# Schatten2021/rust-raytracing

Measured on AMD Instinct MI355X. Metric: Mrays/s (primary rays, whole node), 10k-sphere 1080p 64spp, higher is better.
Workload: dtype f64; 1 GPU; C2: 10k random spheres (scene seed 1), 1920x1080, 64 spp; width=1920, height=1080, rays_per_pixel=64, n_objects=10000, partition=single GPU

## Files before the change

rust-raytracing_amd/csrc/rtx_api.hip:

```cpp
#include "../../include/rtx_hip.h"
#include "rtx_launch.h"

#include <cmath>
#include <cstdio>
#include <cstdlib>
#include <cstring>
#include <string>
#include <thread>
#include <vector>

using namespace rtx;

namespace {

thread_local std::string g_last_error;

int32_t fail(RtxStatus st, const std::string &msg)
{
    g_last_error = msg;
    return (int32_t)st;
}

#define RTX_HIP_CHECK(expr)                                                                              \
    do {                                                                                                 \
        hipError_t e_ = (expr);                                                                          \
        if (e_ != hipSuccess)                                                                            \
            return fail(e_ == hipErrorOutOfMemory ? RTX_ERR_OUT_OF_MEMORY : RTX_ERR_HIP,                 \
                        std::string(#expr) + ": " + hipGetErrorString(e_));                              \
    } while (0)

bool device_is_gfx950(int dev)
{
    hipDeviceProp_t prop;
    if (hipGetDeviceProperties(&prop, dev) != hipSuccess) return false;
    return std::strncmp(prop.gcnArchName, "gfx950", 6) == 0;
}

int usable_device_count()
{
    int n = 0;
    if (hipGetDeviceCount(&n) != hipSuccess) { (void)hipGetLastError(); return 0; }
    int ok = 0;
    for (int d = 0; d < n; ++d) ok += device_is_gfx950(d) ? 1 : 0;
    return ok;
}

constexpr size_t kDefaultScratchBytes = (size_t)24576 << 20;

uint32_t tri_leaf_size(bool plain, uint32_t tuning)
{
    const uint32_t t = (tuning >> RTX_TUNE_TRI_LEAF_SHIFT) & 15u;
    const uint32_t v = t ? t : (plain ? 5u : 2u);
    return v > kQNodeLeafMax ? kQNodeLeafMax : v;
}

bool debug_prints()
{
    static const bool on = std::getenv("RTX_HIP_DEBUG") != nullptr;
    return on;
}

}

#ifndef RTX_GRABS_PER_WAVE
#define RTX_GRABS_PER_WAVE 16
#endif

constexpr uint64_t kHalvesBelowRays = 0;

struct RtxSceneHandle_ {
    int device = 0;
    int n_cus = 0;
    RtxConfig cfg{};
    RtxCamera cam{};
    SceneView sv{};
    std::vector<RtxObject> objects;
    std::vector<void *> scene_allocs;
    double *samples = nullptr;  size_t samples_bytes = 0;
    double *acc = nullptr;      size_t acc_bytes = 0;
    double *tables = nullptr;   size_t tables_doubles = 0;
    double *h_tables = nullptr; size_t h_tables_doubles = 0;
    double *state = nullptr;    size_t state_bytes = 0;
    void *wf_state = nullptr;   size_t wf_bytes = 0;
    void *pool = nullptr;       size_t pool_bytes = 0;
    void *slots = nullptr;      size_t slots_bytes = 0;
    void *tile_lists = nullptr; size_t tile_lists_bytes = 0;
    PathStep *transcript = nullptr; uint32_t *transcript_counts = nullptr; uint32_t transcript_steps = 0;
    Counters *counters = nullptr;
    unsigned long long *work_counter = nullptr;
    SceneView *d_sv = nullptr;  bool sv_dirty = true;
    RowsView *d_rv = nullptr;
    hipEvent_t ev[4] = { nullptr, nullptr, nullptr, nullptr };
    struct SecondHalf {
        hipStream_t stream = nullptr;
        hipEvent_t fork = nullptr, join = nullptr, stage1_done = nullptr;
        Counters *counters = nullptr, *counters_stage1 = nullptr;
        unsigned long long *work_counter = nullptr;
        RowsView *d_rv = nullptr;
        double *state = nullptr;    size_t state_bytes = 0;
        void *queue = nullptr;      size_t queue_bytes = 0;
    } half2;
    Counters *counters_stage1 = nullptr;
    size_t scratch_limit = 0;
    hipStream_t last_stream = nullptr;
    bool have_last_stream = false;
    hipEvent_t ev_done = nullptr;
    bool have_done = false;
    unsigned long long *h_watchdog = nullptr;
    hipEvent_t ev_watchdog = nullptr;
    bool watchdog_pending = false;
    uint32_t t_w = 0, t_h = 0, t_rb = 0, t_rs = 0, t_blk = 0, t_nr = 0;
    double t_fov = 0.0;
    bool t_valid = false;
};

namespace {

template <class T>
int32_t upload_vec(RtxSceneHandle_ *h, const std::vector<T> &v, const T **out)
{
    *out = nullptr;
    if (v.empty()) return RTX_OK;
    void *d = nullptr;
    RTX_HIP_CHECK(hipMalloc(&d, v.size() * sizeof(T)));
    h->scene_allocs.push_back(d);
    RTX_HIP_CHECK(hipMemcpy(d, v.data(), v.size() * sizeof(T), hipMemcpyHostToDevice));
    *out = static_cast<const T *>(d);
    return RTX_OK;
}

// ... 573 lines not shown
    hipStream_t stream = static_cast<hipStream_t>(stream_);
    if (stats) std::memset(stats, 0, sizeof *stats);
    if (n_rows == 0 || width == 0) return RTX_OK;
    if (!d_out_rgb) return fail(RTX_ERR_INVALID_ARGUMENT, "rtx_render_rows: null output");
    if ((uint64_t)n_rows * width > 0xFFFFFFF0ull) return fail(RTX_ERR_INVALID_ARGUMENT, "rtx_render_rows: more than 2^32 pixels per call");
    RTX_HIP_CHECK(hipSetDevice(h->device));
    if (int32_t rc = check_watchdog(h, false)) return rc;
    if (int32_t rc = adopt_stream(h, stream)) return rc;
    struct DoneGuard {
        RtxSceneHandle_ *h; hipStream_t stream;
        ~DoneGuard() {
            if (hipEventRecord(h->ev_done, stream) == hipSuccess) h->have_done = true;
            else { (void)hipGetLastError(); (void)hipDeviceSynchronize(); h->have_done = false; }
        }
    } done_guard{h, stream};

    const uint32_t npix = n_rows * width;
    const uint64_t spp = h->cfg.rays_per_pixel;
    if (h->sv.n_objects == 0 && spp > 0) {
        RTX_HIP_CHECK(hipMemsetAsync(d_out_rgb, 0, (size_t)npix * 3 * sizeof(double), stream));
        if (stats) {
            RTX_HIP_CHECK(hipStreamSynchronize(stream));
            stats->primary_rays = (uint64_t)npix * spp;
            stats->kernel = h->cfg.kernel;
        }
        return RTX_OK;
    }
    const uint64_t outside_tree = ((h->sv.bvh_flags & 1u) ? 0u : h->sv.n_spheres) +
                                  (uint64_t)(h->sv.n_tri_filter - h->sv.n_tri_tree);
    uint32_t kernel = h->cfg.kernel;
    const uint32_t tuning = h->cfg.tuning;
    const bool want_tiles = (tuning & RTX_TUNE_NO_TILES) == 0u, classic = (tuning & RTX_TUNE_BVH_CLASSIC) != 0u;
    if (kernel == RTX_KERNEL_AUTO) {
        if (h->sv.n_bvh_nodes != 0 && outside_tree <= 64) {
            const bool mesh = (h->sv.bvh_flags & 2u) != 0u && h->sv.n_tri_tree >= 1024u;
            kernel = mesh ? RTX_KERNEL_BVH_REGROUP : RTX_KERNEL_BVH;
            if (mesh && (uint64_t)npix * spp >= (1ull << 20) && want_tiles && wavefront_mesh_supported(h->sv, true))
                kernel = RTX_KERNEL_WAVEFRONT;
        } else {
            kernel = RTX_KERNEL_MIXED;
        }
    }

#ifndef RTX_LAB
    if (kernel == RTX_KERNEL_BVH || kernel == RTX_KERNEL_BVH_REGROUP || kernel == RTX_KERNEL_WAVEFRONT) {
        const bool sphere_tree = h->sv.n_bvh_nodes != 0 && (h->sv.bvh_flags & 19u) == 17u;
        const bool tri_tree = h->sv.n_bvh_nodes != 0 && (h->sv.bvh_flags & 2u) != 0u;
        if (sphere_tree) kernel = RTX_KERNEL_BVH;
        else if (!tri_tree) kernel = RTX_KERNEL_MIXED;
        else if (kernel == RTX_KERNEL_BVH) kernel = RTX_KERNEL_BVH_REGROUP;
    }
#endif
    const bool wf_mesh = wavefront_mesh_supported(h->sv, want_tiles);
    const bool wf_spheres = kLabBuild && !wf_mesh && h->sv.n_bvh_nodes != 0 && (h->sv.bvh_flags & 3u) == 1u;
    if (kernel == RTX_KERNEL_WAVEFRONT && !wf_mesh && !wf_spheres) kernel = RTX_KERNEL_BVH_REGROUP;
    const bool tiled = (kernel == RTX_KERNEL_BVH || kernel == RTX_KERNEL_BVH_REGROUP || kernel == RTX_KERNEL_WAVEFRONT) && want_tiles;
    const uint32_t tiles_x = tiled ? (width + 7u) / 8u : 0u;
    const uint64_t per_sample64 = tiled ? (uint64_t)tiles_x * ((n_rows + 7u) / 8u) * 64u : (uint64_t)npix;
    if (per_sample64 > 0xFFFFFFF0ull) return fail(RTX_ERR_INVALID_ARGUMENT, "rtx_render_rows: more than 2^32 ray slots per sample");
    const uint32_t per_sample = (uint32_t)per_sample64;
    uint64_t batch = spp;
    uint64_t tile_list_bytes = 0;
    {
        const bool sph2 = kernel == RTX_KERNEL_BVH && (h->sv.bvh_flags & 2u) == 0u && h->sv.n_bvh_nodes != 0;
        const uint64_t per_ray = 4 * sizeof(double) + (kernel == RTX_KERNEL_WAVEFRONT ? wavefront_state_bytes(1u << 20, 1) >> 20 : 0) +
                                 (sph2 ? 64 + 5 : 0);
        size_t cap_bytes = h->scratch_limit ? h->scratch_limit : kDefaultScratchBytes;
        size_t free_b = 0, total_b = 0;
        if (hipMemGetInfo(&free_b, &total_b) == hipSuccess) {
            const size_t mine = h->samples_bytes + h->wf_bytes + h->tile_lists_bytes;
            const size_t avail = (free_b + mine) / 4 * 3;
            if (cap_bytes > avail) cap_bytes = avail;
        } else (void)hipGetLastError();
        if ((tuning & RTX_TUNE_NO_TILE_LISTS) == 0u && tiled) {
            if (sph2) tile_list_bytes = bvh_spheres_tile_list_bytes(per_sample64);
            else if (kernel == RTX_KERNEL_WAVEFRONT && wf_mesh) tile_list_bytes = wavefront_tile_list_bytes(per_sample64);
            if (tile_list_bytes > cap_bytes / 4) tile_list_bytes = 0;
        }
        const uint64_t fixed = tile_list_bytes +
                               (sph2 ? (uint64_t)bvh_spheres_queue_bytes(0, h->n_cus) + bvh_spheres_spill_bytes(h->sv, h->n_cus) : 0) +
                               (kernel == RTX_KERNEL_WAVEFRONT ? (uint64_t)wavefront_state_bytes(0, 1) + wavefront_spill_bytes(h->sv, h->n_cus) : 0) +
                               (kernel == RTX_KERNEL_MIXED || kernel == RTX_KERNEL_MIXED_VERIFY ? (uint64_t)mixed_state_bytes(h->n_cus) : 0);
        const uint64_t room = cap_bytes > fixed ? cap_bytes - fixed : 0;
        const uint64_t fit = room / (per_sample64 * per_ray);
        const uint64_t fit32 = 0xFFFFFFF0ull / per_sample64;
        if (batch > fit) batch = fit ? fit : 1;
        if (batch > fit32) batch = fit32;
    }

    if (int32_t rc = ensure_tables(h, width, height, row_begin, row_stride, row_block, n_rows, stream)) return rc;

    if (spp > 0) {
        if (int32_t rc = grow((void **)&h->samples, &h->samples_bytes, (size_t)(batch * per_sample64 * 4 * sizeof(double)))) return rc;
    }
    if (batch < spp) {
        if (int32_t rc = grow((void **)&h->acc, &h->acc_bytes, (size_t)npix * 3 * sizeof(double))) return rc;
    }
    const bool spheres_kernel = kernel == RTX_KERNEL_BVH && (h->sv.bvh_flags & 2u) == 0u && h->sv.n_bvh_nodes != 0 && !classic;
    const bool mesh_kernel = kernel == RTX_KERNEL_BVH_REGROUP && (h->sv.bvh_flags & 2u) != 0u && !classic;
#ifdef RTX_LAB
    const bool pool_kernel = kernel == RTX_KERNEL_BVH_REGROUP && (h->sv.bvh_flags & 3u) == 1u && h->sv.n_bvh_nodes != 0 && !classic;
#endif
    if (kernel == RTX_KERNEL_BVH || kernel == RTX_KERNEL_BVH_REGROUP) {
#ifdef RTX_LAB
        const size_t need = pool_kernel ? bvh_spheres_pool_bytes(h->sv, h->n_cus)
                            : spheres_kernel ? bvh_spheres_spill_bytes(h->sv, h->n_cus)
                            : mesh_kernel ? bvh_mesh_spill_bytes(h->sv, h->n_cus) : bvh_spill_bytes(h->sv, h->n_cus);
#else
        if (!spheres_kernel && !mesh_kernel) return fail(RTX_ERR_HIP, "internal: no tree kernel for this scene (product dispatch)");
        const size_t need = spheres_kernel ? bvh_spheres_spill_bytes(h->sv, h->n_cus) : bvh_mesh_spill_bytes(h->sv, h->n_cus);
#endif
        if (int32_t rc = grow((void **)&h->state, &h->state_bytes, need)) return rc;
    }
    if (kernel == RTX_KERNEL_MIXED || kernel == RTX_KERNEL_MIXED_VERIFY) {
        if (int32_t rc = grow((void **)&h->state, &h->state_bytes, mixed_state_bytes(h->n_cus))) return rc;
    }
    const bool spheres_two_stage = spheres_kernel && h->cfg.max_bounces > 0 && (tuning & RTX_TUNE_ONE_STAGE) == 0u &&
                                   (batch * per_sample64 >= (1ull << 20) || (tuning & RTX_TUNE_TWO_STAGE) != 0u) &&
                                   bvh_spheres_two_stage_ok(h->sv, tiled);
#ifdef RTX_LAB
    const bool stage2_slots = spheres_two_stage && (tuning & RTX_TUNE_STAGE2_SLOTS) != 0u && (h->sv.bvh_flags & 16u) != 0u &&
                              (tuning & (RTX_TUNE_NO_QNODES | RTX_TUNE_INLINE_LEAVES | RTX_TUNE_STAGE2_POOL | RTX_TUNE_STAGE2_PAIR)) == 0u;
    if (stage2_slots) {
        if (int32_t rc = grow(&h->slots, &h->slots_bytes, bvh_spheres_slots_bytes(h->n_cus))) return rc;
    }
#else
    const bool stage2_slots = false;
#endif
    if (spheres_two_stage) {
        if (int32_t rc = grow(&h->wf_state, &h->wf_bytes, bvh_spheres_queue_bytes(batch * per_sample64, h->n_cus))) return rc;
        if (tile_list_bytes != 0)
            if (int32_t rc = grow(&h->tile_lists, &h->tile_lists_bytes, (size_t)tile_list_bytes)) return rc;
#ifdef RTX_LAB
        if (tuning & (RTX_TUNE_STAGE2_POOL | RTX_TUNE_STAGE2_PAIR)) {
            const size_t a = bvh_spheres_pool2_bytes(h->n_cus), b = bvh_spheres_pair_bytes(h->n_cus);
            if (int32_t rc = grow(&h->pool, &h->pool_bytes, a > b ? a : b)) return rc;
        }
#endif
    }
    if (kernel == RTX_KERNEL_WAVEFRONT) {
#ifdef RTX_LAB
        const size_t need = wf_mesh ? wavefront_spill_bytes(h->sv, h->n_cus) : wavefront_spheres_spill_bytes(h->sv, h->n_cus);
#else
        const size_t need = wavefront_spill_bytes(h->sv, h->n_cus);
#endif
        if (int32_t rc = grow((void **)&h->state, &h->state_bytes, need)) return rc;
        if (int32_t rc = grow(&h->wf_state, &h->wf_bytes, wavefront_state_bytes(batch * per_sample64, wavefront_levels(h->sv)))) return rc;
        if (wf_mesh && tile_list_bytes != 0)
            if (int32_t rc = grow(&h->tile_lists, &h->tile_lists_bytes, (size_t)tile_list_bytes)) return rc;
    }

    RowsView rv{};
    rv.width = width; rv.height = height;
    rv.row_begin = row_begin; rv.row_stride = row_stride; rv.n_rows = n_rows; rv.row_block = row_block;
    rv.npix = npix;
    rv.div_width = make_fastdiv(width); rv.div_row_block = make_fastdiv(row_block); rv.div_npix = make_fastdiv(npix);
    rv.div_tiles_x = make_fastdiv(tiles_x); rv.div_per_sample = make_fastdiv(per_sample);
    rv.sin_x = h->tables; rv.cos_x = h->tables + width;
    rv.sin_y = h->tables + 2 * (size_t)width; rv.cos_y = rv.sin_y + n_rows;

    if (h->sv_dirty) {
        RTX_HIP_CHECK(hipMemcpyAsync(h->d_sv, &h->sv, sizeof(SceneView), hipMemcpyHostToDevice, stream));
        h->sv_dirty = false;
    }
    RTX_HIP_CHECK(hipMemsetAsync(h->counters, 0, sizeof(Counters) * kCounterShards, stream));
    float trace_ms = 0.f, resolve_ms = 0.f, stage1_ms = 0.f;
    unsigned long long s1_exact = 0, s1_filter = 0, s1_box = 0, prev_exact = 0, prev_filter = 0, prev_box = 0;
    uint32_t launches = 0;

    if (spp == 0) {
        rv.n_samples = 0; rv.n_rays = 0; rv.tiles_x = 0;
        RTX_HIP_CHECK(launch_resolve(nullptr, nullptr, d_out_rgb, rv, npix, 0, true, true, stream));
    }
    const uint32_t sph_flags = ((tuning & RTX_TUNE_NO_PACKETS) ? 1u : 0u) | ((tuning & RTX_TUNE_SORT_SURVIVORS) ? 2u : 0u) |
                               ((tuning & RTX_TUNE_STAGE2_POOL) ? 4u : 0u) | ((tuning & RTX_TUNE_STAGE2_PAIR) ? 8u : 0u);
#ifdef RTX_LAB
    const bool halves_can = spheres_two_stage && batch == spp && spp >= 2 && !stage2_slots &&
                            (tuning & (RTX_TUNE_STAGE2_POOL | RTX_TUNE_STAGE2_PAIR)) == 0u;
#else
    const bool halves_can = spheres_two_stage && batch == spp && spp >= 2;
#endif
    const bool halves = halves_can && (tuning & RTX_TUNE_NO_HALVES) == 0u &&
                        ((tuning & RTX_TUNE_HALVES) != 0u || per_sample64 * spp <= kHalvesBelowRays);
    if (halves) {
        auto &b = h->half2;
        if (!b.stream) {
            int least = 0, greatest = 0;
            RTX_HIP_CHECK(hipDeviceGetStreamPriorityRange(&least, &greatest));
            RTX_HIP_CHECK(hipStreamCreateWithPriority(&b.stream, hipStreamNonBlocking, least));
            RTX_HIP_CHECK(hipEventCreateWithFlags(&b.fork, hipEventDisableTiming));
            RTX_HIP_CHECK(hipEventCreateWithFlags(&b.join, hipEventDisableTiming));
            RTX_HIP_CHECK(hipEventCreate(&b.stage1_done));
            RTX_HIP_CHECK(hipMalloc((void **)&b.counters, sizeof(Counters) * kCounterShards));
            RTX_HIP_CHECK(hipMalloc((void **)&b.counters_stage1, sizeof(Counters) * kCounterShards));
            RTX_HIP_CHECK(hipMalloc((void **)&b.work_counter, sizeof(unsigned long long)));
            RTX_HIP_CHECK(hipMalloc((void **)&b.d_rv, sizeof(RowsView)));
        }
        const uint64_t ns[2] = { (spp + 1) / 2, spp / 2 };
        if (int32_t rc = grow((void **)&b.state, &b.state_bytes, bvh_spheres_spill_bytes(h->sv, h->n_cus))) return rc;
        if (int32_t rc = grow(&b.queue, &b.queue_bytes, bvh_spheres_queue_bytes(ns[1] * per_sample64, h->n_cus))) return rc;
        struct Join {
            RtxSceneHandle_ *h; hipStream_t main; bool forked = false;
            ~Join() {
                if (!forked) return;
                if (hipEventRecord(h->half2.join, h->half2.stream) != hipSuccess || hipStreamWaitEvent(main, h->half2.join, 0) != hipSuccess) {
                    (void)hipGetLastError(); (void)hipStreamSynchronize(h->half2.stream);
                }
            }
        } join{h, stream};
        RTX_HIP_CHECK(hipMemsetAsync(b.counters, 0, sizeof(Counters) * kCounterShards, stream));
        if (stats) RTX_HIP_CHECK(hipEventRecord(h->ev[0], stream));
        RTX_HIP_CHECK(hipEventRecord(b.fork, stream));
        RTX_HIP_CHECK(hipStreamWaitEvent(b.stream, b.fork, 0));
        join.forked = true;
        RowsView rvk[2] = { rv, rv };
        for (int k = 0; k < 2; ++k) {
            RowsView &r = rvk[k];
            r.sample_begin = k == 0 ? 0u : (uint32_t)ns[0];
            r.n_samples = (uint32_t)ns[k];
            r.n_rays = per_sample64 * ns[k];
            r.tiles_x = tiles_x;
            const uint64_t per_wave = r.n_rays / ((uint64_t)h->n_cus * 16u * (RTX_GRABS_PER_WAVE / 2));
            r.grab = (uint32_t)(per_wave >= 512 ? 512 : (per_wave <= 64 ? 64 : (per_wave & ~(uint64_t)63)));
            hipStream_t st = k == 0 ? stream : b.stream;
            RTX_HIP_CHECK(hipMemcpyAsync(k == 0 ? h->d_rv : b.d_rv, &r, sizeof(RowsView), hipMemcpyHostToDevice, st));
            RTX_HIP_CHECK(hipMemsetAsync(k == 0 ? h->work_counter : b.work_counter, 0, sizeof(unsigned long long), st));
            RTX_HIP_CHECK(launch_trace_bvh_spheres(h->d_sv, h->sv, k == 0 ? h->d_rv : b.d_rv, r,
                                                   h->samples + (k == 0 ? 0 : (size_t)(per_sample64 * ns[0]) * 4), k == 0 ? h->counters : b.counters,
                                                   k == 0 ? h->work_counter : b.work_counter, reinterpret_cast<uint32_t *>(k == 0 ? h->state : b.state),
                                                   h->n_cus, k == 0 ? h->wf_state : b.queue, sph_flags, st,
                                                   stats ? (k == 0 ? h->counters_stage1 : b.counters_stage1) : nullptr,
                                                   stats ? (k == 0 ? h->ev[3] : b.stage1_done) : nullptr, nullptr, nullptr,
                                                   nullptr, false));
        }
        RTX_HIP_CHECK(hipEventRecord(b.join, b.stream));
        RTX_HIP_CHECK(hipStreamWaitEvent(stream, b.join, 0));
        join.forked = false;
        launches = 1;
        if (stats) RTX_HIP_CHECK(hipEventRecord(h->ev[1], stream));
        rv.sample_begin = 0; rv.n_samples = (uint32_t)spp; rv.n_rays = per_sample64 * spp; rv.tiles_x = tiles_x;
        RTX_HIP_CHECK(launch_resolve(h->samples, h->acc, d_out_rgb, rv, per_sample, spp, true, true, stream));
        if (stats) {
            RTX_HIP_CHECK(hipEventRecord(h->ev[2], stream));
            RTX_HIP_CHECK(hipEventSynchronize(h->ev[2]));
            RTX_HIP_CHECK(hipEventElapsedTime(&trace_ms, h->ev[0], h->ev[1]));
            RTX_HIP_CHECK(hipEventElapsedTime(&resolve_ms, h->ev[1], h->ev[2]));
            float c0 = 0.f, c1 = 0.f;
            RTX_HIP_CHECK(hipEventElapsedTime(&c0, h->ev[0], h->ev[3]));
            RTX_HIP_CHECK(hipEventElapsedTime(&c1, h->ev[0], b.stage1_done));
            stage1_ms = c0 > c1 ? c0 : c1;
            for (Counters *snap : { h->counters_stage1, b.counters_stage1 }) {
                Counters s1[kCounterShards];
                RTX_HIP_CHECK(hipMemcpy(s1, snap, sizeof s1, hipMemcpyDeviceToHost));
                for (int k = 0; k < kCounterShards; ++k) { s1_exact += s1[k].exact_tests; s1_filter += s1[k].filter_tests; if (k >= 2) s1_box += s1[k].pad_; }
            }
        }
    }
    for (uint64_t s0 = 0; s0 < spp && !halves; s0 += batch) {
        const uint64_t ns = (spp - s0 < batch) ? spp - s0 : batch;
        rv.sample_begin = (uint32_t)s0;
        rv.n_samples = (uint32_t)ns;
        rv.n_rays = per_sample64 * ns;
        rv.tiles_x = tiles_x;
        {
            const uint64_t per_wave = rv.n_rays / ((uint64_t)h->n_cus * 16u * RTX_GRABS_PER_WAVE);
            rv.grab = (uint32_t)(per_wave >= 512 ? 512 : (per_wave <= 64 ? 64 : (per_wave & ~(uint64_t)63)));
        }
        RTX_HIP_CHECK(hipMemcpyAsync(h->d_rv, &rv, sizeof(RowsView), hipMemcpyHostToDevice, stream));
        if (stats) RTX_HIP_CHECK(hipEventRecord(h->ev[0], stream));
        if (kernel == RTX_KERNEL_EXACT) {
            RTX_HIP_CHECK(launch_trace_exact(h->d_sv, h->d_rv, rv, h->samples, h->counters, stream));
#ifdef RTX_LAB
            if (h->transcript)
                RTX_HIP_CHECK(launch_trace_transcript(h->d_sv, h->d_rv, rv, h->transcript, h->transcript_counts, h->transcript_steps, stream));
#endif
        } else if (kernel == RTX_KERNEL_WAVEFRONT) {
#ifdef RTX_LAB
            if (!wf_mesh)
                RTX_HIP_CHECK(launch_trace_wavefront_spheres(h->d_sv, h->sv, h->d_rv, rv, h->samples, h->wf_state, h->counters,
                                                             reinterpret_cast<uint32_t *>(h->state), h->n_cus, stream));
            else
#endif
                RTX_HIP_CHECK(launch_trace_wavefront(h->d_sv, h->sv, h->d_rv, rv, h->samples, h->wf_state, h->counters,
                                                     reinterpret_cast<uint32_t *>(h->state), h->n_cus, stream,
                                                     wf_mesh && tile_list_bytes != 0 ? h->tile_lists : nullptr, s0 == 0));
        } else if (kernel == RTX_KERNEL_BVH_REGROUP) {
            RTX_HIP_CHECK(hipMemsetAsync(h->work_counter, 0, sizeof(unsigned long long), stream));
#ifdef RTX_LAB
            if (pool_kernel)
                RTX_HIP_CHECK(launch_trace_bvh_spheres_pool(h->d_sv, h->sv, h->d_rv, rv, h->samples, h->counters, h->work_counter,
                                                            h->state, h->n_cus, stream));
            else if (!mesh_kernel)
                RTX_HIP_CHECK(launch_trace_bvh_regroup(h->d_sv, h->sv, h->d_rv, rv, h->samples, h->counters, h->work_counter,
                                                       reinterpret_cast<uint32_t *>(h->state), h->n_cus, stream));
            else
#endif
                RTX_HIP_CHECK(launch_trace_bvh_mesh(h->d_sv, h->sv, h->d_rv, rv, h->samples, h->counters, h->work_counter,
                                                    reinterpret_cast<uint32_t *>(h->state), h->n_cus, stream));
        } else if (kernel == RTX_KERNEL_BVH) {
            RTX_HIP_CHECK(hipMemsetAsync(h->work_counter, 0, sizeof(unsigned long long), stream));
#ifdef RTX_LAB
            if (!spheres_kernel)
                RTX_HIP_CHECK(launch_trace_bvh(h->d_sv, h->sv, h->d_rv, rv, h->samples, h->counters, h->work_counter,
                                               reinterpret_cast<uint32_t *>(h->state), h->n_cus, stream));
            else
#endif
                RTX_HIP_CHECK(launch_trace_bvh_spheres(h->d_sv, h->sv, h->d_rv, rv, h->samples, h->counters, h->work_counter,
                                                       reinterpret_cast<uint32_t *>(h->state), h->n_cus,
                                                       spheres_two_stage ? h->wf_state : nullptr, sph_flags, stream,
                                                       stats && spheres_two_stage ? h->counters_stage1 : nullptr,
                                                       stats && spheres_two_stage ? h->ev[3] : nullptr, spheres_two_stage && (tuning & (RTX_TUNE_STAGE2_POOL | RTX_TUNE_STAGE2_PAIR)) ? h->pool : nullptr,
                                                       stage2_slots ? h->slots : nullptr,
                                                       spheres_two_stage && tile_list_bytes != 0 ? h->tile_lists : nullptr, s0 == 0));
        } else {
            RTX_HIP_CHECK(hipMemsetAsync(h->work_counter, 0, sizeof(unsigned long long), stream));
            RTX_HIP_CHECK(launch_trace_mixed(h->d_sv, h->sv, h->d_rv, rv, h->samples, h->state, h->counters, h->work_counter, h->n_cus,
                                             kernel == RTX_KERNEL_MIXED_VERIFY, stream));
        }
        ++launches;
        if (stats) RTX_HIP_CHECK(hipEventRecord(h->ev[1], stream));
        RTX_HIP_CHECK(launch_resolve(h->samples, h->acc, d_out_rgb, rv, per_sample, spp, s0 == 0, s0 + ns == spp, stream));
        if (stats) {
            RTX_HIP_CHECK(hipEventRecord(h->ev[2], stream));
            RTX_HIP_CHECK(hipEventSynchronize(h->ev[2]));
            float a = 0.f, b = 0.f;
            RTX_HIP_CHECK(hipEventElapsedTime(&a, h->ev[0], h->ev[1]));
            RTX_HIP_CHECK(hipEventElapsedTime(&b, h->ev[1], h->ev[2]));
            trace_ms += a; resolve_ms += b;
            if (spheres_two_stage) {
                float c = 0.f;
                RTX_HIP_CHECK(hipEventElapsedTime(&c, h->ev[0], h->ev[3]));
                stage1_ms += c;
                Counters s1[kCounterShards];
                RTX_HIP_CHECK(hipMemcpy(s1, h->counters_stage1, sizeof s1, hipMemcpyDeviceToHost));
                unsigned long long e1 = 0, f1 = 0, b1 = 0;
                for (int k = 0; k < kCounterShards; ++k) { e1 += s1[k].exact_tests; f1 += s1[k].filter_tests; if (k >= 2) b1 += s1[k].pad_; }
                Counters now[kCounterShards];
                RTX_HIP_CHECK(hipMemcpy(now, h->counters, sizeof now, hipMemcpyDeviceToHost));
                unsigned long long e2 = 0, f2 = 0, b2 = 0;
                for (int k = 0; k < kCounterShards; ++k) { e2 += now[k].exact_tests; f2 += now[k].filter_tests; if (k >= 2) b2 += now[k].pad_; }
                s1_exact += e1 - prev_exact; s1_filter += f1 - prev_filter; s1_box += b1 - prev_box;
                prev_exact = e2; prev_filter = f2; prev_box = b2;
            }
        }
    }
    if (kernel == RTX_KERNEL_MIXED || kernel == RTX_KERNEL_MIXED_VERIFY || spheres_two_stage) {
        if (h->watchdog_pending) RTX_HIP_CHECK(hipEventSynchronize(h->ev_watchdog));
        if (int32_t rc = check_watchdog(h, false)) return rc;
        RTX_HIP_CHECK(hipMemcpyAsync(h->h_watchdog, &h->counters[1].pad_, sizeof(unsigned long long), hipMemcpyDeviceToHost, stream));
        if (halves) RTX_HIP_CHECK(hipMemcpyAsync(h->h_watchdog + 1, &h->half2.counters[1].pad_, sizeof(unsigned long long), hipMemcpyDeviceToHost, stream));
        RTX_HIP_CHECK(hipEventRecord(h->ev_watchdog, stream));
// ... 539 lines not shown
```

rust-raytracing_amd/csrc/rtx_device.h:

```cpp
#pragma once

#include "rtx_bvh.h"
#include "rtx_scene.h"

namespace rtx {

struct SceneView {
    uint64_t rays_per_pixel;
    uint64_t max_bounces;
    double   focal_length, focal_offset, non_focal_offset;
    uint64_t seed;
    V3 cam_pos;
    V3 to_world_x, to_world_y, to_world_z;
    uint32_t n_objects, n_spheres, n_planes, n_tris;
    const SphereX  *spheres;
    const uint32_t *sphere_id;
    const PlaneX   *planes;
    const TriX     *tris;
    const MaterialX *materials;
    const float4   *tri_f32;
    const uint32_t *tri_fidx;
    const float4   *tri_geo;
    uint32_t        n_tri_filter;
    uint32_t        pad0_;
    double          tri_extent;
    const float4   *sphere_f32;
    double          sphere_center[3];
    double          sphere_cmax;
    const Bvh4Node *bvh_nodes;
    const BvhQNode *bvh_qnodes;
    const BvhQ3Node *bvh_q3nodes;
    const uint32_t *bvh_prims;
    const float4   *bvh_leaf_f32;
    const float4   *bvh_leaf_cr;
    uint32_t        n_bvh_nodes;
    uint32_t        bvh_root;
    uint32_t        bvh_depth;
    uint32_t        tuning;
    float           bvh_origin_limit;
    uint32_t        bvh_flags;
    uint32_t        n_tri_tree;
    float           bvh_inv_max;
};

struct FastDiv { uint32_t m, s1, s2, d; };

inline FastDiv make_fastdiv(uint32_t d)
{
    FastDiv f;
    f.d = d ? d : 1u;
    uint32_t l = 0;
    while (l < 32u && (1ull << l) < (unsigned long long)f.d) ++l;
    f.m = (uint32_t)((((1ull << l) - (unsigned long long)f.d) << 32) / (unsigned long long)f.d + 1ull);
    f.s1 = l < 1u ? l : 1u;
    f.s2 = l > 1u ? l - 1u : 0u;
    return f;
}

RTX_HD uint32_t fastdiv(uint32_t n, const FastDiv &f)
{
#if defined(__HIP_DEVICE_COMPILE__)
    const uint32_t t = __umulhi(f.m, n);
#else
    const uint32_t t = (uint32_t)(((unsigned long long)f.m * (unsigned long long)n) >> 32);
#endif
    return (t + ((n - t) >> f.s1)) >> f.s2;
}

struct RowsView {
    uint32_t width, height;
    uint32_t row_begin, row_stride, n_rows;
    uint32_t row_block;
    uint32_t npix;
    uint32_t sample_begin;
    uint32_t n_samples;
    uint64_t n_rays;
    uint32_t grab;
    uint32_t tiles_x;
    const double *sin_x, *cos_x, *sin_y, *cos_y;
    FastDiv div_width, div_row_block, div_npix, div_tiles_x, div_per_sample;
};

RTX_HD uint32_t image_row(const RowsView &rv, uint32_t k)
{
    const uint32_t b = fastdiv(k, rv.div_row_block);
    return rv.row_begin + b * rv.row_stride + (k - b * rv.row_block);
}

struct PathStep {
    double pos[3], dir[3], t;
    long long object;
};

struct Counters {
    unsigned long long segments;
    unsigned long long exact_tests;
    unsigned long long filter_tests;
    unsigned long long pad_;
};
constexpr int kCounterShards = 64;

struct RayState {
    V3 pos, dir, result, light;
    uint64_t key;
    uint32_t draw;
    uint32_t bounce;
};

struct Hit {
    double   t;
    uint32_t id;
    uint32_t kind;
    uint32_t local;
};

__device__ __forceinline__ void hit_init(Hit &h) { h.t = 0.0; h.id = 0xFFFFFFFFu; h.kind = 0; h.local = 0; }

__device__ __forceinline__ void hit_consider(Hit &h, double t, uint32_t id, uint32_t kind, uint32_t local)
{
    if (!is_normal_positive(t)) return;
    if (h.id == 0xFFFFFFFFu || t < h.t || (t == h.t && id < h.id)) { h.t = t; h.id = id; h.kind = kind; h.local = local; }
}

__device__ __forceinline__ void ray_index_to_pixel(const RowsView &rv, uint64_t i, uint32_t &pl, uint32_t &s_local)
{
    s_local = fastdiv((uint32_t)i, rv.div_npix);
    pl = (uint32_t)i - s_local * rv.npix;
}

__device__ __forceinline__ bool ray_index_to_pixel_tiled(const RowsView &rv, uint64_t i, uint32_t &pl, uint32_t &s_local)
{
    s_local = fastdiv((uint32_t)i, rv.div_per_sample);
    const uint32_t r = (uint32_t)i - s_local * rv.div_per_sample.d;
    const uint32_t t = r >> 6, j = r & 63u;
    const uint32_t ty = fastdiv(t, rv.div_tiles_x), tx = t - ty * rv.tiles_x;
    const uint32_t x = tx * 8u + (j & 7u), k = ty * 8u + (j >> 3);
    pl = k * rv.width + x;
    return x < rv.width && k < rv.n_rows;
}

__device__ __forceinline__ void store_sample(double *__restrict__ samples, const RowsView &rv, uint64_t ridx, V3 c)
{
    (void)rv;
    double4 *rec = reinterpret_cast<double4 *>(samples) + ridx;
    *rec = make_double4(c.x, c.y, c.z, 0.0);
}

__device__ __forceinline__ V3 primary_focal_point(const SceneView &sv, const RowsView &rv, uint32_t pl)
{
    const uint32_t k = fastdiv(pl, rv.div_width);
    const uint32_t x = pl - k * rv.width;
    const V3 cam_space_dir = mk(rv.sin_x[x], rv.sin_y[k], rv.cos_x[x] * rv.cos_y[k]);
    const V3 ray_dir = mk(dot(cam_space_dir, sv.to_world_x), dot(cam_space_dir, sv.to_world_y),
                          dot(cam_space_dir, sv.to_world_z));
    return vadd(sv.cam_pos, vmuls(ray_dir, sv.focal_length));
}

__device__ __forceinline__ float round_down_f32_dev(double x)
{
    float f = (float)x;
    if ((double)f > x) f = __uint_as_float(f > 0.0f ? __float_as_uint(f) - 1u : (f < 0.0f ? __float_as_uint(f) + 1u : 0x80000001u));
    return f;
}

__device__ __forceinline__ void gen_primary(const SceneView &sv, const RowsView &rv, uint32_t pl, uint32_t sample,
                                            RayState &r)
{
    uint32_t k = fastdiv(pl, rv.div_width);
    uint32_t x = pl - k * rv.width;
    uint32_t y = image_row(rv, k);
    uint64_t pix = (uint64_t)y * rv.width + x;
    r.key = rng_key(sv.seed, pix, sample);
    V3 rnd1;
    rnd1.x = rng_u01(r.key, 0); rnd1.y = rng_u01(r.key, 1); rnd1.z = rng_u01(r.key, 2);
    V3 ray_position = vadd(sv.cam_pos, vmuls(rnd1, sv.non_focal_offset));
    V3 focal_point = primary_focal_point(sv, rv, pl);
    V3 rnd2;
    rnd2.x = rng_u01(r.key, 3); rnd2.y = rng_u01(r.key, 4); rnd2.z = rng_u01(r.key, 5);
    V3 target_point = vadd(focal_point, vmuls(rnd2, sv.focal_offset));
    V3 ray_direction = vsub(target_point, ray_position);
    r.pos = ray_position;
    r.dir = vnorm(ray_direction);
    r.result = mk(0.0, 0.0, 0.0);
    r.light = mk(1.0, 1.0, 1.0);
    r.draw = 6;
    r.bounce = 0;
}

__device__ __forceinline__ V3 random_direction(double u_z, double u_theta)
{
    double z = u_z * 2.0 - 1.0;
    double theta = u_theta * 2.0 * 3.14159265358979323846;
    double r = sqrt(1.0 - z * z);
    double sn, cs;
    sincos_2pi(theta, &sn, &cs);
    return vnorm(mk(r * cs, r * sn, z));
}

__device__ __forceinline__ V3 random_bounce_dir(V3 ray_dir, V3 surface_normal, double surface_roughness,
                                                double u_z, double u_theta)
{
    V3 random_dir = random_direction(u_z, u_theta);
    V3 reflection_dir = vsub(ray_dir, vmuls(vmuls(surface_normal, 2.0), dot(ray_dir, surface_normal)));
    V3 random_to_reflection_dir = vsub(reflection_dir, random_dir);
    double reflection_mult = 1.0 - surface_roughness;
    V3 final_direction = vadd(random_dir, vmuls(random_to_reflection_dir, reflection_mult));
    final_direction = vnorm(final_direction);
    if (dot(final_direction, surface_normal) > 0.0) return final_direction;
    return vneg(final_direction);
}

__device__ __forceinline__ V3 normal_at(const SceneView &sv, const Hit &h, V3 world_pos)
{
    if (h.kind == 0) return sphere_normal_at(sv.spheres[h.local], world_pos);
    if (h.kind == 1) return sv.planes[h.local].nhat;
    return sv.tris[h.local].nn;
}

__device__ __forceinline__ void advance_and_shade(const SceneView &sv, const Hit &h, RayState &r)
{
    r.pos = vadd(r.pos, vmuls(r.dir, h.t));
    const MaterialX m = sv.materials[h.id];
    double u_z = rng_u01(r.key, r.draw);
    double u_theta = rng_u01(r.key, r.draw + 1);
    r.draw += 2;
    r.dir = random_bounce_dir(r.dir, normal_at(sv, h, r.pos), m.roughness, u_z, u_theta);
    r.result = vadd(r.result, vmulv(r.light, m.emission_color));
    r.light = vmulv(r.light, m.base_color);
// ... 85 lines not shown
```

rust-raytracing_amd/csrc/rtx_kernels.hip:

```cpp
#include "rtx_launch.h"
#include "rtx_traverse.h"

#include <cstdlib>

namespace rtx {

__device__ __forceinline__ uint32_t lane_id() { return __builtin_amdgcn_mbcnt_hi(~0u, __builtin_amdgcn_mbcnt_lo(~0u, 0u)); }

__device__ __forceinline__ uint32_t mbcnt(unsigned long long mask)
{
    return __builtin_amdgcn_mbcnt_hi((uint32_t)(mask >> 32), __builtin_amdgcn_mbcnt_lo((uint32_t)mask, 0u));
}

__device__ __forceinline__ unsigned long long wave_sum_u64(unsigned long long v)
{
#pragma unroll
    for (int off = 32; off > 0; off >>= 1) v += __shfl_xor(v, off, 64);
    return v;
}

__device__ __forceinline__ void flush_counters(Counters *ctr, unsigned long long segs, unsigned long long exact,
                                               unsigned long long filt)
{
    segs = wave_sum_u64(segs);
// ... 348 lines not shown
            r.dir = mk(st[3 * n_slots], st[4 * n_slots], st[5 * n_slots]);
            const RayX rx = make_rayx(r.pos, r.dir);
            Hit h;
            hit_init(h);
            ++segs;
            if (ncand > (uint32_t)(Q + kOverflowQ)) {
                closest_spheres_exact(sv, rx, h);
                closest_tris_exact(sv, rx, h);
                exact += ns + sv.n_tris;
            } else {
                for (uint32_t k = 0; k < ncand; ++k) {
                    const uint32_t idx = k < (uint32_t)Q ? lds_q[((size_t)k * S + s) * THREADS + tid]
                                                         : oflow[(size_t)(k - Q) * n_slots + slot];
                    double t;
                    if (idx & 0x80000000u) {
                        const uint32_t ti = idx & 0x7FFFFFFFu;
                        if (ti < sv.n_tris && triangle_distance(sv.tris[ti], rx, &t)) hit_consider(h, t, sv.tris[ti].id, 2, ti);
                    } else if (idx < ns) {
                        if (sphere_distance(sv.spheres[idx], rx, &t)) hit_consider(h, t, sv.sphere_id[idx], 0, idx);
                    }
                }
                exact += ncand;
                if (verify) {
                    Hit hv;
                    hit_init(hv);
                    closest_spheres_exact(sv, rx, hv);
                    closest_tris_exact(sv, rx, hv);
                    if (hv.id != h.id || (hv.id != kInvalid && hv.t != h.t)) {
                        ++mism;
                        if (verify > 1 && mism < 3)
                            printf("MISMATCH round %llu bnc %u pl %u blk %u tid %u s %d ncand %u h(%u,%g) hv(%u,%g) pos(%g,%g,%g) "
                                   "dir(%g,%g,%g)\n", round, bnc, pl, blockIdx.x, tid, s, ncand, h.id, h.t, hv.id, hv.t, r.pos.x,
                                   r.pos.y, r.pos.z, r.dir.x, r.dir.y, r.dir.z);
                    }
                }
            }
            closest_planes_exact(sv, rx, h);
            exact += sv.n_planes;

            r.result = mk(st[6 * n_slots], st[7 * n_slots], st[8 * n_slots]);
            bool done = true;
            if (h.id != kInvalid) {
                r.light = mk(st[9 * n_slots], st[10 * n_slots], st[11 * n_slots]);
                const uint32_t k = fastdiv(pl, rv.div_width);
                const uint32_t x = pl - k * rv.width;
                const uint64_t pix = (uint64_t)image_row(rv, k) * rv.width + x;
                r.key = rng_key(sv.seed, pix, rv.sample_begin + smp);
                r.draw = 6u + 2u * bnc;
                r.bounce = bnc;
                advance_and_shade(sv, h, r);
                done = (r.bounce >= bounce_limit) || light_is_zero(r);
                if (!done) {
                    st[0 * n_slots] = r.pos.x; st[1 * n_slots] = r.pos.y; st[2 * n_slots] = r.pos.z;
                    st[3 * n_slots] = r.dir.x; st[4 * n_slots] = r.dir.y; st[5 * n_slots] = r.dir.z;
                    st[6 * n_slots] = r.result.x; st[7 * n_slots] = r.result.y; st[8 * n_slots] = r.result.z;
                    st[9 * n_slots] = r.light.x; st[10 * n_slots] = r.light.y; st[11 * n_slots] = r.light.z;
                    is[2 * n_slots] = r.bounce;
                    FilterParams f;
                    filter_from_ray(sv, r.pos, r.dir, f);
                    float *fs = fstate + slot;
                    fs[0 * n_slots] = f.dx; fs[1 * n_slots] = f.dy; fs[2 * n_slots] = f.dz; fs[3 * n_slots] = f.npd;
                    fs[4 * n_slots] = f.p2x; fs[5 * n_slots] = f.p2y; fs[6 * n_slots] = f.p2z; fs[7 * n_slots] = f.nppE;
                    {
                        TriFilterParams tf;
                        if (sv.n_tri_filter != 0) tri_filter_from_ray(sv, r.pos, r.dir, tf); else tri_filter_idle(tf);
                        fs[8 * n_slots] = tf.dx; fs[9 * n_slots] = tf.dy; fs[10 * n_slots] = tf.dz; fs[11 * n_slots] = tf.npx;
                        fs[12 * n_slots] = tf.npy; fs[13 * n_slots] = tf.npz; fs[14 * n_slots] = tf.A;
                    }
                }
            }
            if (done) {
                store_sample(samples, rv, (uint64_t)smp * rv.npix + pl, r.result);
                live &= ~(1u << s);
            }
        }
    }
    flush_counters(ctr, segs, exact, rounds_swept * ((unsigned long long)ns + sv.n_tri_filter) * S);
    if (verify) {
        mism = wave_sum_u64(mism);
        if (lane == 0 && mism) atomicAdd(&ctr[0].pad_, mism);
    }
}

__global__ __launch_bounds__(256) void resolve_kernel(const double *__restrict__ samples, double *__restrict__ acc,
                                                      double *__restrict__ out, uint32_t width, uint32_t n_rows, uint32_t tiles_x,
                                                      uint32_t per_sample, uint32_t n_samples,
                                                      double divisor, int first, int last)
{
    const uint32_t t = blockIdx.x * blockDim.x + threadIdx.x;
    if (t >= per_sample) return;
    uint32_t p = t;
    if (tiles_x != 0u) {
        const uint32_t tile = t >> 6, j = t & 63u;
        const uint32_t ty = tile / tiles_x, tx = tile - ty * tiles_x;
        const uint32_t x = tx * 8u + (j & 7u), k = ty * 8u + (j >> 3);
        if (x >= width || k >= n_rows) return;
        p = k * width + x;
    }
    double sx = 0.0, sy = 0.0, sz = 0.0;
    if (!first) { sx = acc[3 * (uint64_t)p]; sy = acc[3 * (uint64_t)p + 1]; sz = acc[3 * (uint64_t)p + 2]; }
    for (uint32_t s = 0; s < n_samples; ++s) {
        const double4 c = reinterpret_cast<const double4 *>(samples)[(uint64_t)s * per_sample + t];
        sx = sx + c.x; sy = sy + c.y; sz = sz + c.z;
    }
    if (last) {
        double *o = out + 3 * (uint64_t)p;
        o[0] = sx / divisor; o[1] = sy / divisor; o[2] = sz / divisor;
    } else {
        acc[3 * (uint64_t)p] = sx; acc[3 * (uint64_t)p + 1] = sy; acc[3 * (uint64_t)p + 2] = sz;
    }
}

__device__ __forceinline__ uint8_t rust_as_u8(double v)
{
    if (!(v == v)) return 0;
    if (v <= 0.0) return 0;
    if (v >= 255.0) return 255;
    return (uint8_t)v;
}

__global__ __launch_bounds__(256) void quantize_kernel(const double *__restrict__ rgb, uint8_t *__restrict__ rgb8,
                                                       uint32_t width, uint32_t height, uint32_t flip)
{
    uint64_t p = (uint64_t)blockIdx.x * blockDim.x + threadIdx.x;
    uint64_t npix = (uint64_t)width * height;
    if (p >= npix) return;
    uint32_t y = (uint32_t)(p / width);
    uint32_t x = (uint32_t)(p - (uint64_t)y * width);
    const double *c = rgb + 3 * ((uint64_t)(flip ? height - y - 1 : y) * width + x);
    uint8_t *o = rgb8 + 3 * p;
    o[0] = rust_as_u8(c[0] * 256.0);
    o[1] = rust_as_u8(c[1] * 256.0);
    o[2] = rust_as_u8(c[2] * 256.0);
}

__global__ __launch_bounds__(256) void deinterleave_kernel(const uint8_t *__restrict__ parts, uint8_t *__restrict__ full,
                                                           uint32_t width, uint32_t height, uint32_t n, uint32_t cap_rows,
                                                           uint32_t block, uint32_t flip, uint32_t elem_bytes)
{
    const uint64_t i = (uint64_t)blockIdx.x * blockDim.x + threadIdx.x;
    const uint64_t row_vals = (uint64_t)width * 3;
    if (i >= row_vals * height) return;
    const uint32_t yo = (uint32_t)(i / row_vals);
    const uint64_t c = i - (uint64_t)yo * row_vals;
    const uint32_t y = flip ? height - 1u - yo : yo;
    const uint32_t b = y / block, p = b % n, k = (b / n) * block + (y - b * block);
    const uint64_t src = ((uint64_t)p * cap_rows + k) * row_vals + c;
    if (elem_bytes == 8u) reinterpret_cast<unsigned long long *>(full)[i] = reinterpret_cast<const unsigned long long *>(parts)[src];
    else full[i] = parts[src];
}

#ifdef RTX_LAB
__global__ void debug_math_kernel(int op, const double *a, const double *b, double *out, uint64_t n, RowsView rv)
{
    uint64_t i = (uint64_t)blockIdx.x * blockDim.x + threadIdx.x;
    if (i >= n) return;
    double r;
    switch (op) {
        case 0: r = a[i] / b[i]; break;
        case 1: r = sqrt(a[i]); break;
        case 2: r = sin(a[i]); break;
        case 3: r = cos(a[i]); break;
        case 4: case 5: { double sn, cs; sincos(a[i], &sn, &cs); r = (op == 4) ? sn : cs; } break;
        case 6:
            r = (double)rtx_writelane(__builtin_amdgcn_readfirstlane((int)b[0]), __builtin_amdgcn_readfirstlane((int)b[1]), (int)a[i]);
            break;
        case 9: case 10: { double sn, cs; sincos_2pi(a[i], &sn, &cs); r = (op == 9) ? sn : cs; } break;
        case 11: r = (double)fastdiv((uint32_t)a[i], rv.div_npix); break;
        case 12: case 13: {
            uint32_t pl, s_local;
            ray_index_to_pixel(rv, (uint64_t)a[i], pl, s_local);
            r = (double)(op == 12 ? pl : s_local);
        } break;
        case 14: case 15: case 16: {
            uint32_t pl, s_local;
            const bool live = ray_index_to_pixel_tiled(rv, (uint64_t)a[i], pl, s_local);
            r = op == 14 ? (double)pl : (op == 15 ? (double)s_local : (live ? 1.0 : 0.0));
        } break;
        default: {
            double lo, hi;
            rtx_minmax_f64_bits(a[i], b[i], lo, hi);
            r = (op == 7) ? lo : hi;
        } break;
    }
    out[i] = r;
}
// ... 16 lines not shown
namespace {

struct MixVariant {
    int s, threads, chunk, q, blocks_per_cu;
    size_t lds;
    const void *fn;
};

template <int S, int T, int CH, int Q, int WPE, int BPC>
MixVariant make_variant()
{
    MixVariant v;
    v.s = S; v.threads = T; v.chunk = CH; v.q = Q; v.blocks_per_cu = BPC;
    v.lds = (size_t)CH * 16 + (size_t)Q * S * T * 4 + (size_t)S * T * 4 + (T / 64 + 4) * 4;
    v.fn = reinterpret_cast<const void *>(&trace_mixed_kernel<S, T, CH, Q, WPE>);
    return v;
}

const MixVariant &mix_variant()
{
    static const MixVariant table[] = {
        make_variant<2, 256, 1024, 8, 4, 4>(),
#ifdef RTX_MIXED_TUNING
        make_variant<2, 512, 2048, 8, 4, 2>(),
        make_variant<3, 256, 1024, 8, 3, 3>(),
        make_variant<4, 256, 2048, 8, 2, 2>(),
        make_variant<1, 512, 1024, 8, 8, 4>(),
        make_variant<2, 1024, 2048, 8, 4, 1>(),
        make_variant<4, 256, 2048, 8, 4, 2>(),
        make_variant<2, 256, 2048, 8, 4, 3>(),
        make_variant<2, 128, 1024, 8, 4, 8>(),
#endif
    };
#ifdef RTX_MIXED_TUNING
    static const int idx = [] {
        const char *e = getenv("RTX_HIP_MIXED_VARIANT");
        int i = e ? atoi(e) : 0;
        return (i < 0 || i >= (int)(sizeof(table) / sizeof(table[0]))) ? 0 : i;
    }();
    return table[idx];
#else
    return table[0];
#endif
}

}

size_t mixed_state_bytes(int n_cus)
{
    const MixVariant &v = mix_variant();
    return (size_t)n_cus * v.blocks_per_cu * v.threads * v.s * kSlotBytes;
}

hipError_t launch_trace_mixed(const SceneView *d_sv, const SceneView &sv, const RowsView *d_rv, const RowsView &rv,
                              double *samples, double *state, Counters *counters, unsigned long long *work_counter,
                              int n_cus, bool verify, hipStream_t stream)
{
    const MixVariant &v = mix_variant();
    {
        hipError_t e = hipFuncSetAttribute(v.fn, hipFuncAttributeMaxDynamicSharedMemorySize, (int)v.lds);
        if (e != hipSuccess) return e;
    }
    const uint64_t slots_per_block = (uint64_t)v.threads * v.s;
    uint64_t want = (rv.n_rays + slots_per_block - 1) / slots_per_block;
    uint64_t cap = (uint64_t)n_cus * v.blocks_per_cu;
    uint32_t blocks = (uint32_t)(want < cap ? want : cap);
    if (blocks == 0) return hipSuccess;
    const unsigned long long limit = sv.max_bounces >= 0xFFFFFFF0ull ? 0xFFFFFFF0ull : sv.max_bounces + 1ull;
    unsigned long long max_rounds = (rv.n_rays / slots_per_block + 2ull) * limit + 4ull;
#ifdef RTX_MIXED_TUNING
    uint32_t verify_u = verify ? (getenv("RTX_HIP_DEBUG_PRINT") ? 2u : 1u) : 0u;
#else
    uint32_t verify_u = verify ? 1u : 0u;
#endif
    void *args[] = { (void *)&d_sv, (void *)&d_rv, (void *)&samples, (void *)&state, (void *)&counters, (void *)&work_counter,
                     (void *)&verify_u, (void *)&max_rounds };
    return hipLaunchKernel(v.fn, dim3(blocks), dim3(v.threads), args, v.lds, stream);
}

hipError_t launch_resolve(const double *samples, double *acc, double *out, const RowsView &rv, uint32_t per_sample,
                          uint64_t rays_per_pixel, bool first, bool last, hipStream_t stream)
{
    if (per_sample == 0) return hipSuccess;
    hipLaunchKernelGGL(resolve_kernel, dim3((per_sample + 255) / 256), dim3(256), 0, stream, samples, acc, out, rv.width, rv.n_rows,
                       rv.tiles_x, per_sample, rv.n_samples, (double)rays_per_pixel, first ? 1 : 0, last ? 1 : 0);
    return hipGetLastError();
}

hipError_t launch_quantize(const double *rgb, uint8_t *rgb8, uint32_t width, uint32_t height, hipStream_t stream)
{
    uint64_t npix = (uint64_t)width * height;
    if (npix == 0) return hipSuccess;
    hipLaunchKernelGGL(quantize_kernel, dim3((uint32_t)((npix + 255) / 256)), dim3(256), 0, stream, rgb, rgb8, width,
                       height, 1u);
    return hipGetLastError();
}

hipError_t launch_quantize_values(const double *rgb, uint8_t *rgb8, uint32_t width, uint32_t n_rows, hipStream_t stream)
{
    uint64_t npix = (uint64_t)width * n_rows;
    if (npix == 0) return hipSuccess;
    hipLaunchKernelGGL(quantize_kernel, dim3((uint32_t)((npix + 255) / 256)), dim3(256), 0, stream, rgb, rgb8, width,
                       n_rows, 0u);
    return hipGetLastError();
}

hipError_t launch_deinterleave(const double *parts, double *full, uint32_t width, uint32_t height, uint32_t n, uint32_t cap_rows,
                               uint32_t block, hipStream_t stream)
{
    const uint64_t total = (uint64_t)width * height * 3;
    if (total == 0) return hipSuccess;
    hipLaunchKernelGGL(deinterleave_kernel, dim3((uint32_t)((total + 255) / 256)), dim3(256), 0, stream,
                       reinterpret_cast<const uint8_t *>(parts), reinterpret_cast<uint8_t *>(full), width, height, n, cap_rows, block, 0u, 8u);
    return hipGetLastError();
}

hipError_t launch_deinterleave_u8(const uint8_t *parts, uint8_t *full, uint32_t width, uint32_t height, uint32_t n, uint32_t cap_rows,
                                  uint32_t block, bool flip, hipStream_t stream)
{
    const uint64_t total = (uint64_t)width * height * 3;
    if (total == 0) return hipSuccess;
    hipLaunchKernelGGL(deinterleave_kernel, dim3((uint32_t)((total + 255) / 256)), dim3(256), 0, stream, parts, full, width,
                       height, n, cap_rows, block, flip ? 1u : 0u, 1u);
    return hipGetLastError();
}

#ifdef RTX_LAB
static RowsView debug_index_view(int op, const double *b_host, uint64_t n)
{
    RowsView rv{};
    const uint32_t b0 = b_host ? (uint32_t)b_host[0] : 0u, b1 = (b_host && n > 1) ? (uint32_t)b_host[1] : 0u;
    if (op >= 11 && op <= 13) {
        rv.npix = b0;
        rv.div_npix = make_fastdiv(b0);
    } else if (op >= 14 && op <= 16) {
        rv.width = b0; rv.n_rows = b1; rv.npix = b0 * b1;
        rv.tiles_x = (b0 + 7u) / 8u;
        rv.div_width = make_fastdiv(b0); rv.div_npix = make_fastdiv(rv.npix); rv.div_tiles_x = make_fastdiv(rv.tiles_x);
        rv.div_per_sample = make_fastdiv((uint32_t)((uint64_t)rv.tiles_x * ((b1 + 7u) / 8u) * 64u));
    }
    return rv;
}

hipError_t launch_debug_math(int op, const double *a, const double *b, double *out, uint64_t n, const double *b_host, hipStream_t stream)
{
    if (n == 0) return hipSuccess;
    hipLaunchKernelGGL(debug_math_kernel, dim3((uint32_t)((n + 255) / 256)), dim3(256), 0, stream, op, a, b, out, n,
                       debug_index_view(op, b_host, n));
    return hipGetLastError();
}

bool debug_math_host(int op, const double *a, const double *b, double *out, uint64_t n)
{
    if (op < 17 || op > 21) return false;
    RowsView rv{};
    if (op == 18) {
        if (n < 3) return false;
        rv.row_begin = (uint32_t)b[0]; rv.row_stride = (uint32_t)b[1]; rv.row_block = (uint32_t)b[2];
        rv.div_row_block = make_fastdiv(rv.row_block);
    }
    const FastDiv f17 = make_fastdiv((uint32_t)b[0]);
    for (uint64_t i = 0; i < n; ++i) {
        const uint32_t v = (uint32_t)a[i];
        const FastDiv f = make_fastdiv(v);
        out[i] = op == 17 ? (double)fastdiv(v, f17) : op == 18 ? (double)image_row(rv, v) : op == 19 ? (double)f.m : op == 20 ? (double)f.s1 : (double)f.s2;
    }
    return true;
// ... 5 lines not shown
```

Measured before the change: 3771 Mrays/s.

## Skip storing black samples and track nonzero samples with a bitmask

Trace kernels no longer write all-zero (black) sample colors and instead set a bit in a per-ray nonzero bitmask via atomicOr. The resolve kernel reads the bitmask eight samples at a time and loads only the samples whose bit is set, which cuts write and read traffic on the sample buffer when many rays miss. In exchange it adds a memset of the mask per batch, global atomics on every nonzero store, and extra bitmask loads in resolve. The batch-fit computation is adjusted to reserve room for the mask.

Result: faster. 3913 Mrays/s, median of 6 (+3.8%).

```diff
diff --git a/rust-raytracing_amd/csrc/rtx_api.hip b/rust-raytracing_amd/csrc/rtx_api.hip
--- a/rust-raytracing_amd/csrc/rtx_api.hip
+++ b/rust-raytracing_amd/csrc/rtx_api.hip
@@ -46,6 +46,8 @@
 }
 
 constexpr size_t kDefaultScratchBytes = (size_t)24576 << 20;
+
+static size_t nonzero_mask_bytes(uint64_t n_rays) { return (size_t)((n_rays + 31) / 32) * sizeof(uint32_t); }
 
 uint32_t tri_leaf_size(bool plain, uint32_t tuning)
 {
@@ -785,7 +787,7 @@
                                (kernel == RTX_KERNEL_WAVEFRONT ? (uint64_t)wavefront_state_bytes(0, 1) + wavefront_spill_bytes(h->sv, h->n_cus) : 0) +
                                (kernel == RTX_KERNEL_MIXED || kernel == RTX_KERNEL_MIXED_VERIFY ? (uint64_t)mixed_state_bytes(h->n_cus) : 0);
         const uint64_t room = cap_bytes > fixed ? cap_bytes - fixed : 0;
-        const uint64_t fit = room / (per_sample64 * per_ray);
+        const uint64_t fit = room * 8 / (per_sample64 * (per_ray * 8 + 1));
         const uint64_t fit32 = 0xFFFFFFF0ull / per_sample64;
         if (batch > fit) batch = fit ? fit : 1;
         if (batch > fit32) batch = fit32;
@@ -794,7 +796,8 @@
     if (int32_t rc = ensure_tables(h, width, height, row_begin, row_stride, row_block, n_rows, stream)) return rc;
 
     if (spp > 0) {
-        if (int32_t rc = grow((void **)&h->samples, &h->samples_bytes, (size_t)(batch * per_sample64 * 4 * sizeof(double)))) return rc;
+        if (int32_t rc = grow((void **)&h->samples, &h->samples_bytes,
+                              (size_t)(batch * per_sample64 * 4 * sizeof(double)) + nonzero_mask_bytes(batch * per_sample64))) return rc;
     }
     if (batch < spp) {
         if (int32_t rc = grow((void **)&h->acc, &h->acc_bytes, (size_t)npix * 3 * sizeof(double))) return rc;
@@ -861,6 +864,8 @@
     rv.div_tiles_x = make_fastdiv(tiles_x); rv.div_per_sample = make_fastdiv(per_sample);
     rv.sin_x = h->tables; rv.cos_x = h->tables + width;
     rv.sin_y = h->tables + 2 * (size_t)width; rv.cos_y = rv.sin_y + n_rows;
+    rv.nonzero = spp > 0 ? reinterpret_cast<uint32_t *>(h->samples + (size_t)(batch * per_sample64) * 4) : nullptr;
+    rv.nonzero_base = 0;
 
     if (h->sv_dirty) {
         RTX_HIP_CHECK(hipMemcpyAsync(h->d_sv, &h->sv, sizeof(SceneView), hipMemcpyHostToDevice, stream));
@@ -912,6 +917,7 @@
             }
         } join{h, stream};
         RTX_HIP_CHECK(hipMemsetAsync(b.counters, 0, sizeof(Counters) * kCounterShards, stream));
+        RTX_HIP_CHECK(hipMemsetAsync(rv.nonzero, 0, nonzero_mask_bytes(per_sample64 * spp), stream));
         if (stats) RTX_HIP_CHECK(hipEventRecord(h->ev[0], stream));
         RTX_HIP_CHECK(hipEventRecord(b.fork, stream));
         RTX_HIP_CHECK(hipStreamWaitEvent(b.stream, b.fork, 0));
@@ -922,6 +928,7 @@
             r.sample_begin = k == 0 ? 0u : (uint32_t)ns[0];
             r.n_samples = (uint32_t)ns[k];
             r.n_rays = per_sample64 * ns[k];
+            r.nonzero_base = k == 0 ? 0 : per_sample64 * ns[0];
             r.tiles_x = tiles_x;
             const uint64_t per_wave = r.n_rays / ((uint64_t)h->n_cus * 16u * (RTX_GRABS_PER_WAVE / 2));
             r.grab = (uint32_t)(per_wave >= 512 ? 512 : (per_wave <= 64 ? 64 : (per_wave & ~(uint64_t)63)));
@@ -970,6 +977,7 @@
             rv.grab = (uint32_t)(per_wave >= 512 ? 512 : (per_wave <= 64 ? 64 : (per_wave & ~(uint64_t)63)));
         }
         RTX_HIP_CHECK(hipMemcpyAsync(h->d_rv, &rv, sizeof(RowsView), hipMemcpyHostToDevice, stream));
+        RTX_HIP_CHECK(hipMemsetAsync(rv.nonzero, 0, nonzero_mask_bytes(rv.n_rays), stream));
         if (stats) RTX_HIP_CHECK(hipEventRecord(h->ev[0], stream));
         if (kernel == RTX_KERNEL_EXACT) {
             RTX_HIP_CHECK(launch_trace_exact(h->d_sv, h->d_rv, rv, h->samples, h->counters, stream));
diff --git a/rust-raytracing_amd/csrc/rtx_device.h b/rust-raytracing_amd/csrc/rtx_device.h
--- a/rust-raytracing_amd/csrc/rtx_device.h
+++ b/rust-raytracing_amd/csrc/rtx_device.h
@@ -78,6 +78,8 @@
     uint32_t grab;
     uint32_t tiles_x;
     const double *sin_x, *cos_x, *sin_y, *cos_y;
+    uint32_t *nonzero;
+    uint64_t nonzero_base;
     FastDiv div_width, div_row_block, div_npix, div_tiles_x, div_per_sample;
 };
 
@@ -141,9 +143,11 @@
 
 __device__ __forceinline__ void store_sample(double *__restrict__ samples, const RowsView &rv, uint64_t ridx, V3 c)
 {
-    (void)rv;
+    if (c.x == 0.0 && c.y == 0.0 && c.z == 0.0) return;
     double4 *rec = reinterpret_cast<double4 *>(samples) + ridx;
     *rec = make_double4(c.x, c.y, c.z, 0.0);
+    const uint64_t bit = rv.nonzero_base + ridx;
+    atomicOr(rv.nonzero + (bit >> 5), 1u << (uint32_t)(bit & 31u));
 }
 
 __device__ __forceinline__ V3 primary_focal_point(const SceneView &sv, const RowsView &rv, uint32_t pl)
diff --git a/rust-raytracing_amd/csrc/rtx_kernels.hip b/rust-raytracing_amd/csrc/rtx_kernels.hip
--- a/rust-raytracing_amd/csrc/rtx_kernels.hip
+++ b/rust-raytracing_amd/csrc/rtx_kernels.hip
@@ -454,7 +454,8 @@
     }
 }
 
-__global__ __launch_bounds__(256) void resolve_kernel(const double *__restrict__ samples, double *__restrict__ acc,
+__global__ __launch_bounds__(256) void resolve_kernel(const double *__restrict__ samples, const uint32_t *__restrict__ nonzero,
+                                                      double *__restrict__ acc,
                                                       double *__restrict__ out, uint32_t width, uint32_t n_rows, uint32_t tiles_x,
                                                       uint32_t per_sample, uint32_t n_samples,
                                                       double divisor, int first, int last)
@@ -471,9 +472,27 @@
     }
     double sx = 0.0, sy = 0.0, sz = 0.0;
     if (!first) { sx = acc[3 * (uint64_t)p]; sy = acc[3 * (uint64_t)p + 1]; sz = acc[3 * (uint64_t)p + 2]; }
-    for (uint32_t s = 0; s < n_samples; ++s) {
-        const double4 c = reinterpret_cast<const double4 *>(samples)[(uint64_t)s * per_sample + t];
-        sx = sx + c.x; sy = sy + c.y; sz = sz + c.z;
+    constexpr uint32_t kAhead = 8;
+    for (uint32_t s0 = 0; s0 < n_samples; s0 += kAhead) {
+        const uint32_t n = n_samples - s0 < kAhead ? n_samples - s0 : kAhead;
+        uint32_t set = 0;
+#pragma unroll
+        for (uint32_t j = 0; j < kAhead; ++j) {
+            if (j < n) {
+                const uint64_t slot = (uint64_t)(s0 + j) * per_sample + t;
+                set |= ((nonzero[slot >> 5] >> (uint32_t)(slot & 31u)) & 1u) << j;
+            }
+        }
+        if (set == 0u) continue;
+        double4 c[kAhead];
+#pragma unroll
+        for (uint32_t j = 0; j < kAhead; ++j) {
+            c[j] = make_double4(0.0, 0.0, 0.0, 0.0);
+            if ((set >> j) & 1u) c[j] = reinterpret_cast<const double4 *>(samples)[(uint64_t)(s0 + j) * per_sample + t];
+        }
+#pragma unroll
+        for (uint32_t j = 0; j < kAhead; ++j)
+            if ((set >> j) & 1u) { sx = sx + c[j].x; sy = sy + c[j].y; sz = sz + c[j].z; }
     }
     if (last) {
         double *o = out + 3 * (uint64_t)p;
@@ -656,7 +675,7 @@
                           uint64_t rays_per_pixel, bool first, bool last, hipStream_t stream)
 {
     if (per_sample == 0) return hipSuccess;
-    hipLaunchKernelGGL(resolve_kernel, dim3((per_sample + 255) / 256), dim3(256), 0, stream, samples, acc, out, rv.width, rv.n_rows,
+    hipLaunchKernelGGL(resolve_kernel, dim3((per_sample + 255) / 256), dim3(256), 0, stream, samples, rv.nonzero, acc, out, rv.width, rv.n_rows,
                        rv.tiles_x, per_sample, rv.n_samples, (double)rays_per_pixel, first ? 1 : 0, last ? 1 : 0);
     return hipGetLastError();
 }
```
